# RHnejad/3D_PoseEstimation

Hardware: AMD Instinct MI355X
Metric: poses/sec fwd+bwd, 17-joint lifting batch 4096; MPJPE vs ref (higher is better)
Workload: dtype f16x3 (two fp16 planes per fp32 operand, 3 fp16 MFMAs per product, fp32 accumulate); 1 GPU; BASELINE configs[1]: phase1_lifting LinearModel 34-1024-2x(1024-1024)-51, BN+ReLU+Dropout(0.5), one train_1.py step = zero_grad+forward+MSE+backward+AdamW; launch=hipgraph (one hipGraph replay per step), per_gpu_batch=4096, global_batch=4096, parallelism=dp1

## Files before the change

3d_poseestimation_amd/_lib.py:

```python
import ctypes
import os

import torch

_HERE = os.path.dirname(os.path.abspath(__file__))
LIB_PATH = os.environ.get("POSELIFT_LIB") or os.path.join(_HERE, "csrc", "libposelift.so")

PL_F32, PL_BF16, PL_BF16X6, PL_F16X3 = 0, 1, 2, 3


GATHER_FN = ctypes.CFUNCTYPE(ctypes.c_int, ctypes.c_void_p, ctypes.c_void_p, ctypes.c_int64, ctypes.c_void_p)


class PLSync(ctypes.Structure):
    _fields_ = [("world", ctypes.c_int32), ("rank", ctypes.c_int32), ("gather", GATHER_FN),
                ("user", ctypes.c_void_p)]


class PLL1Term(ctypes.Structure):
    _fields_ = [("a", ctypes.c_void_p), ("b", ctypes.c_void_p), ("n", ctypes.c_int64),
                ("da", ctypes.c_void_p), ("db", ctypes.c_void_p)]


L1_MAX_TERMS = 8
# ... 40 lines not shown
_D = ctypes.POINTER(PLDesc)
SIGNATURES = {
    "pl_version": (_c.c_int, []),
    "pl_last_error": (_c.c_char_p, []),
    "pl_num_hidden": (_c.c_int64, [_D]),
    "pl_param_tensors": (_c.c_int64, [_D]),
    "pl_param_offset": (_c.c_int64, [_D, _c.c_int64]),
    "pl_param_numel": (_c.c_int64, [_D, _c.c_int64]),
    "pl_param_arena_floats": (_c.c_int64, [_D]),
    "pl_workspace_bytes": (_c.c_size_t, [_D, _c.c_int64]),
    "pl_workspace_view": (_c.c_int, [_D, _c.c_int64, _c.c_int, _c.c_int64,
                                     _c.POINTER(_c.c_size_t), _c.POINTER(_c.c_size_t)]),
    "pl_workspace_bitmap_format": (_c.c_int, [_D, _c.c_int64, _c.c_int64]),
    "pl_lifter_fwd_eval": (_c.c_int, [_D, _P, _P, _c.c_int64, _P, _c.c_size_t, _P]),
    "pl_lifter_fwd_train": (_c.c_int, [_D, _P, _P, _c.c_int64, _P, _c.c_size_t, _c.c_uint64,
                                       _c.c_uint64, _P, _P]),
    "pl_lifter_bwd": (_c.c_int, [_D, _P, _P, _c.c_int64, _P, _c.c_size_t, _P, _P, _P]),
    "pl_lifter_fwd_eval_saved": (_c.c_int, [_D, _P, _P, _c.c_int64, _P, _c.c_size_t, _P]),
    "pl_lifter_bwd_eval": (_c.c_int, [_D, _P, _P, _c.c_int64, _P, _c.c_size_t, _P, _P, _P]),
    "pl_lifter_bwd_layers": (_c.c_int, [_D, _P, _P, _c.c_int64, _P, _c.c_size_t, _P, _P, _c.c_int, _c.c_int, _P]),
    "pl_lifter_train_fwd_bwd": (_c.c_int, [_D, _P, _P, _c.c_int64, _P, _c.c_size_t, _c.c_uint64, _c.c_uint64,
                                           _P, _P, _P, _c.c_int, _c.c_int, _P]),
    "pl_lifter_step_carries_adamw": (_c.c_int, [_D, _c.c_int64]),
    "pl_lifter_train_step": (_c.c_int, [_D, _P, _P, _c.c_int64, _P, _c.c_size_t, _c.c_uint64, _c.c_uint64,
                                        _P, _P, _P, _c.POINTER(PLAdamWStep), _P]),
    "pl_mse_scratch_bytes": (_c.c_size_t, [_c.c_int64]),
    "pl_mse_fwd_bwd": (_c.c_int, [_P, _P, _c.c_int64, _c.c_float, _P, _P, _P, _P]),
    "pl_l1_scratch_bytes": (_c.c_size_t, [_c.c_int]),
    "pl_l1_terms_fwd_bwd": (_c.c_int, [_c.POINTER(PLL1Term), _c.c_int, _c.c_float, _P, _P, _P]),
    "pl_mpjpe_scratch_bytes": (_c.c_size_t, [_c.c_int64, _c.c_int64]),
    "pl_mpjpe_accum": (_c.c_int, [_P, _P, _c.c_int64, _c.c_int64, _P, _P, _P]),
    "pl_adamw_flat": (_c.c_int, [_P, _P, _P, _P, _c.c_int64, _c.c_float, _c.c_float, _c.c_float,
                                 _c.c_float, _c.c_float, _c.c_int64, _c.c_float, _P]),
    "pl_adamw_flat_dev": (_c.c_int, [_P, _P, _P, _P, _c.c_int64, _P, _c.c_float, _c.c_float, _c.c_float,
                                     _c.c_float, _c.c_int64, _P, _c.c_float, _P]),
    "pl_adamw_flat_planes": (_c.c_int, [_P, _P, _P, _P, _c.c_int64, _c.c_float, _P, _c.c_float, _c.c_float, _c.c_float,
                                        _c.c_float, _c.c_int64, _P, _c.c_float, _c.POINTER(PLAdamWPlanes), _P]),
    "pl_wplanes_bytes": (_c.c_size_t, [_D]),
    "pl_wplanes_layer_bytes": (_c.c_size_t, [_D]),
    "pl_weight_plane_scale": (_c.c_float, []),
    "pl_wplanes_refresh": (_c.c_int, [_D, _P]),
    "pl_flip_pose": (_c.c_int, [_P, _P, _c.c_int64, _c.c_int64, _c.c_int64, _P]),
    "pl_counter_add": (_c.c_int, [_P, _c.c_int64, _P]),
    "pl_flip_pose_ex": (_c.c_int, [_P, _P, _P, _c.c_int64, _c.c_int64, _c.c_int64, _c.c_float, _c.c_float, _P]),
    "pl_flip_w_nhwc": (_c.c_int, [_P, _P, _c.c_int64, _c.c_int64, _c.c_int64, _c.c_int64, _P]),
    "pl_softargmax3d_nhwc_fwd": (_c.c_int, [_P, _c.c_int64, _c.c_int64, _c.c_int64, _c.c_int64, _P, _P, _P]),
# ... 178 lines not shown
```

3d_poseestimation_amd/csrc/api.hip:

```cpp
#include <stdarg.h>
#include <stdio.h>
#include <stdlib.h>

#include <vector>

#include "adamw.h"
#include "pl_internal.h"

namespace pl {

static thread_local char g_err[512] = "";

void set_error(const char* fmt, ...) {
  va_list ap;
  va_start(ap, fmt);
  vsnprintf(g_err, sizeof(g_err), fmt, ap);
  va_end(ap);
}

namespace {

inline int64_t align_up(int64_t v, int64_t a) { return (v + a - 1) / a * a; }

int check_desc(const PLDesc* d, bool need_arenas) {
// ... 107 lines not shown
  bool bnr_fused;
};
enum class Loss : uint8_t { SmallMse, FromSlabs, PartialOnly };

struct Ws {
  int L, G, RC;
  std::vector<size_t> z, act, bits, mean, rstd, dbpart;
  size_t stat, scale, shift, coef, ga, gb, dz, slabs, outpart, dyout, mse, total;
  size_t act_bytes, bits_bytes;
  size_t slab_floats;
  bool planes;
  int pkind;
  std::vector<size_t> actp, wp;
  std::vector<size_t> sactp;
  std::vector<char> act_f32;
  size_t dzp, amax, dzscale;
  size_t skp_out, skp_in;
  std::vector<size_t> wslab;
  std::vector<LayerRoute> layer;
  bool bn_small;
  bool small_layer;
  bool top_fused;
  bool adam_rides;
  bool small_f16;
  bool eval_small;
  bool out_narrow;
  bool out_skinny;
  Loss loss;
};

Ws plan(const PLDesc* d, int64_t B) {
  Ws w;
  w.L = 1 + 2 * d->num_stage;
  const int H = d->hidden;
  w.G = gemm_stat_groups((int)B);
  w.RC = bwd_row_chunks((int)B, H);
  size_t o = 0;
  auto take = [&](size_t bytes) {
    const size_t at = o;
    o = (size_t)align_up((int64_t)(o + bytes), 256);
    return at;
  };
  w.act_bytes = (size_t)B * H * sizeof(float);
  w.bits_bytes = std::max((size_t)B * bitmap_words_per_row(H), (size_t)H) * sizeof(uint64_t);
  w.pkind = planes_kind(d, B);
  w.planes = w.pkind != 0;
// ... 41 lines not shown
  w.skp_out = take((size_t)skinny_in_chunks((int)B) * d->out_dim * H * 4);
  w.skp_in = take((size_t)skinny_in_chunks((int)B) * d->in_dim * H * 4);
  if (w.planes) {
    w.wslab.push_back(0);
    for (int l = 1; l < w.L; ++l) w.wslab.push_back(take((size_t)tn_splits(H, H, (int)B) * H * H * 4));
    for (int l = 0; l + 1 < w.L; ++l) w.actp.push_back(take(w.act_bytes));
    w.wp.push_back(0);
    for (int l = 1; l < w.L; ++l) w.wp.push_back(take((size_t)H * H * 4));
    w.dzp = take(w.act_bytes);
    w.amax = take(std::max((size_t)((H + 255) / 256) * w.RC, (size_t)(B / 64) * (H / 32)) * 2 * 4);
    w.dzscale = take((size_t)w.L * 2 * 4);
  }
  if (d->dtype == PL_F16X3 && B <= kThinGemmMaxM)
    for (int l = 0; l + 1 < w.L; ++l) w.sactp.push_back(take(w.act_bytes));
  w.total = o;

  const int world = sync_world(d);
  const bool first_ok = small_first_ok(d->in_dim), mid_ok = B * world <= 512 && small_layer_ok(2, H, H);
  w.bn_small = d->bn && !w.planes && world == 1 && B >= 2 && B <= kBnSmallRows;
  w.small_layer = w.bn_small && small_layer_ok((int)B, H, H);
  w.top_fused = w.small_layer && small_top_ok(d->out_dim);
  const bool small_head = w.top_fused && (d->num_stage > 0 || first_ok);
  w.adam_rides = small_head && H % 128 == 0;
  w.small_f16 = d->dtype == PL_F16X3 && !w.sactp.empty() && first_ok;
  w.eval_small = d->bn && B <= kThinGemmMaxM && small_layer_ok(2, H, H) && first_ok && small_top_ok(d->out_dim);
  w.out_narrow = skinny_narrow_out_supported(H, d->out_dim);
  w.out_skinny = skinny_supported(d->out_dim, H);
  const int so = w.out_narrow ? skinny_narrow_out_splits((int)B, H) : 0;
  w.loss = small_head ? Loss::SmallMse : (so && mse_from_slabs_supported(so, d->out_dim)) ? Loss::FromSlabs : Loss::PartialOnly;
  for (int l = 0; l < w.L; ++l) {
    LayerRoute r;
    if (l == 0) r.lin = skinny_supported(d->in_dim, H) ? Lin::Skinny : Lin::Gemm;
    else if (w.planes) r.lin = w.pkind == 2 && mid_ok ? Lin::PlanesMid : Lin::Planes;
    else r.lin = d->bn && d->dtype != PL_BF16 && B > kBnSmallRows && mid_ok ? Lin::F32Mid : Lin::Gemm;
    r.groups = r.lin == Lin::Skinny ? skinny_stat_groups((int)B) : w.G;
    const bool tile = w.small_layer && (l > 0 || first_ok);
    if (!d->bn) r.stats = Stats::None;
    else if (w.bn_small) r.stats = tile ? Stats::InLayer : Stats::Small;
    else r.stats = world == 1 && r.groups >= 1 && r.groups <= 4 ? Stats::InApply : Stats::Finalize;
    if (l == 0) r.bwd = tile && w.L > 1 ? Bwd::InAbove : Bwd::First;
    else if (!w.small_layer) r.bwd = w.planes ? Bwd::PlanesPair : Bwd::F32Pair;
    else r.bwd = H % 128 == 0 ? Bwd::SmallLayerDw : Bwd::SmallLayer;
    r.bnr_fused = w.planes && (l < w.L - 1 || w.out_skinny);
    w.layer.push_back(r);
  }
  return w;
// ... 388 lines not shown
  const int H = d->hidden, O = d->out_dim, Bi = (int)B;
  const float kscale = (!eval_bn && d->p_dropout > 0.f && d->p_dropout < 1.f) ? 1.0f / (1.0f - d->p_dropout) : 1.0f;
  float* slabs = f32(ws, w.slabs);
  float* GA = f32(ws, w.ga);
  float* GB = f32(ws, w.gb);
  float* DZ = f32(ws, w.dz);
  const int64_t BH = B * H;
  const int n_amax = ((H + 255) / 256) * w.RC;
  std::vector<const float*> jpart; std::vector<float*> jout; std::vector<int> jR, jH, jkind, jtrans;
  auto job = [&](const float* part, float* out, int R, int Hj, int kind, int transK) {
    jpart.push_back(part); jout.push_back(out); jR.push_back(R); jH.push_back(Hj); jkind.push_back(kind); jtrans.push_back(transK);
  };

  const bool small = !eval_bn && w.bn_small, sl = !eval_bn && w.small_layer;
  auto bn_layer = [&](int l) {
    const Layer y = layer_of(d, P, grads, l);
    SmallBnLayer b = {f32(ws, w.z[l]), f32(ws, w.mean[l]), f32(ws, w.rstd[l]), y.gamma, u64(ws, w.bits[l]),
                      w.layer[l].stats != Stats::InLayer, y.ggamma, y.gbeta, y.gb};
    return b;
  };
  const int n_loss_part = loss_partials > 0 ? loss_partials : mse_partials(B * O);
  const bool top_fused = do_output && !eval_bn && w.top_fused && l_hi == w.L - 1 && l_hi >= l_lo;
  const bool adam_rides = adam && top_fused && l_lo == 0 && w.adam_rides;
  auto ride = [&](int64_t lo, int64_t hi) {
    AdamWRide r = {};
    r.p = const_cast<float*>(d->params) + lo; r.g = grads + lo; r.m = adam->m + lo; r.v = adam->v + lo; r.n = hi - lo;
    r.lr = adam->lr; r.beta1 = adam->beta1; r.beta2 = adam->beta2; r.eps = adam->eps; r.wd = adam->weight_decay; r.gscale = 1.0f;
    r.t = adam->t; r.lr_dev = adam->lr_dev; r.t_dev = adam->t_dev;
    return r;
  };
  if (top_fused) {
    PL_TRY(launch_small_top_bwd(dy, d->params + P.off[4 * w.L], f32(ws, w.act[w.L - 1]), Bi, H, O, GA, grads + P.off[4 * w.L],
                                grads + P.off[4 * w.L + 1], bn_layer(w.L - 1), kscale, DZ, s, f32(ws, w.mse),
                                n_loss_part, 1.0f / (float)(B * O), loss_out, const_cast<uint64_t*>(d->step_dev)));
  } else if (do_output && w.out_skinny) {
    PL_TRY(launch_skinny_wide_in(dy, f32(ws, w.act[w.L - 1]), grads + P.off[4 * w.L], Bi, O, H, false, f32(ws, w.skp_out), s,
                                 false, f32(ws, w.outpart)));
    job(f32(ws, w.skp_out), grads + P.off[4 * w.L], skinny_in_chunks(Bi), O * H, 0, 0);
    job(f32(ws, w.outpart), grads + P.off[4 * w.L + 1], skinny_in_chunks(Bi), O, 0, 0);
    GemmArgs be = {};
    const int lt = w.L - 1;
    if (!eval_bn && w.layer[lt].bnr_fused) {
      const BnrSlab sl = bnr_slab(d, w, ws, Bi / 64, (w.pkind == 2 && lt > 0) ? (Bi / 64) * (H / 32) : 0, eval_bn);
      be.bnr_z = f32(ws, w.z[lt]); be.bnr_bits = u64(ws, w.bits[lt]);
      be.bnr_mean = f32(ws, w.mean[lt]); be.bnr_rstd = f32(ws, w.rstd[lt]); be.bnr_kscale = kscale;
      be.bnr_part_dy = sl.mine; be.bnr_part_dyz = sl.mine + (size_t)(Bi / 64) * H;
// ... 51 lines not shown
    const float* a_in = l == 0 ? x : (w.planes ? nullptr : f32(ws, w.act[l - 1]));
    if (pl_layer) {
      const int splits = tn_splits(H, H, Bi);
      PlanesGemmArgs nn = planes_args(w.pkind, u16(ws, w.dzp), BH, H, wplane(d, w, ws, l), (int64_t)H * H, H,
                                      (l % 2 == 1) ? GA : GB, Bi, H, H, 1.0f / kWeightPlaneScale, dzs ? dzs + 1 : nullptr);
      if (l % 2 == 1) nn.e.addend = GA;
      if (!eval_bn && w.layer[l - 1].bnr_fused) {
        const bool lower_scaled = w.pkind == 2 && l - 1 > 0;
        const BnrSlab sl = bnr_slab(d, w, ws, Bi / 64, lower_scaled ? (Bi / 64) * (H / 64) : 0, eval_bn);
        nn.e.bnr_z = f32(ws, w.z[l - 1]);
        nn.e.bnr_bits = u64(ws, w.bits[l - 1]);
        nn.e.bnr_mean = f32(ws, w.mean[l - 1]);
        nn.e.bnr_rstd = f32(ws, w.rstd[l - 1]);
        nn.e.bnr_kscale = kscale;
        nn.e.bnr_part_dy = sl.mine;
        nn.e.bnr_part_dyz = sl.mine + (size_t)(Bi / 64) * H;
        nn.e.bnr_amax = lower_scaled ? sl.amax_mine : nullptr;
      }
      float* wsl = f32(ws, w.wslab[l]);
      PlanesGemmArgs tn = planes_args(w.pkind, u16(ws, w.dzp), BH, H, u16(ws, w.actp[l - 1]), BH, H,
                                      splits > 1 ? wsl : ly.gW, H, H, Bi, 1.0f / kActPlaneScale, dzs ? dzs + 1 : nullptr);
      tn.e.split_k = splits;
      PL_TRY(launch_gemm_planes_pair(nn, tn, s));
      if (splits > 1) job(wsl, ly.gW, splits, H * H, 1, 0);
    } else if (l > 0) {
      GemmArgs g = {};
      g.A = DZl; g.B = ly.W; g.M = Bi; g.N = H; g.K = H; g.lda = H; g.ldb = H; g.ldc = H; g.split_k = 1;
      if (l % 2 == 1) { g.C = GA; g.addend = GA; } else { g.C = GB; }
      g.arith = arith_of(d);
      g.thin_scratch = slabs; g.thin_scratch_floats = w.slab_floats;
      GemmArgs t = {};
      t.arith = g.arith;
      t.A = DZl; t.B = a_in; t.M = H; t.N = H; t.K = Bi; t.lda = H; t.ldb = H; t.ldc = H; t.split_k = 1; t.C = ly.gW;
      if (sl && (r.bwd == Bwd::SmallLayer || r.bwd == Bwd::SmallLayerDw)) {
        const bool dw_rides = r.bwd == Bwd::SmallLayerDw;
        if (l - 1 >= l_lo) {
          const bool w1 = l == 1 && w.layer[0].bwd == Bwd::InAbove;
          AdamWRide ar = {};
          if (adam_rides) ar = ride(P.off[4 * l + 1], l == w.L - 1 ? P.total : P.off[4 * (l + 1) + 1]);
          PL_TRY(launch_small_layer_bwd(DZl, ly.W, (l % 2 == 1) ? GA : nullptr, (l % 2 == 1) ? GA : nullptr, Bi, H, H,
                                        bn_layer(l - 1), kscale, dzbuf(l - 1), s, dw_rides ? a_in : nullptr,
                                        dw_rides ? ly.gW : nullptr, w1 ? x : nullptr, w1 ? grads + P.off[0] : nullptr, d->in_dim,
                                        adam_rides ? &ar : nullptr));
          if (dw_rides) continue;
        } else {
          PL_TRY(launch_gemm_f32(kNN, g, s));
        }
// ... 12 lines not shown
      PL_TRY(gemm_tn_reduced(DZ, H, a_in, ly.K, ly.gW, H, ly.K, Bi, slabs, s));
    }
    if (l == 0 && dx) {
      GemmArgs g = {};
      g.A = DZ; g.B = ly.W; g.C = dx; g.M = Bi; g.N = d->in_dim; g.K = H; g.lda = H; g.ldb = d->in_dim;
      g.ldc = d->in_dim; g.split_k = 1;
      PL_TRY(launch_gemm_f32(kNN, g, s));
    }
  }
  float inv_n = 0.f;
  uint64_t* tick = nullptr;
  if (loss_out && !top_fused) {
    const int64_t n = B * O;
    job(f32(ws, w.mse), loss_out, n_loss_part, 1, 2, 0);
    inv_n = 1.0f / (float)n;
    tick = const_cast<uint64_t*>(d->step_dev);
  }
  if (!jpart.empty())
    PL_TRY(launch_reduce_rows_multi(jpart.data(), jR.data(), jH.data(), jout.data(), (int)jpart.size(), s, jkind.data(),
                                    jtrans.data(), inv_n, tick));
  if (adam) {
    const int64_t n = adam_rides ? (w.L > 1 ? P.off[4 * 1 + 1] : P.total) : P.total;
    float* p = const_cast<float*>(d->params);
    if (adam->lr_dev)
      PL_TRY(pl_adamw_flat_dev(p, grads, adam->m, adam->v, n, adam->lr_dev, adam->beta1, adam->beta2, adam->eps,
                               adam->weight_decay, adam->t, adam->t_dev, 1.0f, stream));
    else
      PL_TRY(pl_adamw_flat(p, grads, adam->m, adam->v, n, adam->lr, adam->beta1, adam->beta2, adam->eps, adam->weight_decay,
                           adam->t, 1.0f, stream));
  }
  return PL_OK;
}

extern "C" int pl_lifter_bwd(const PLDesc* d, const float* x, const float* dy, int64_t B, void* ws,
                             size_t ws_bytes, float* dx, float* grads, void* stream) {
  if (!d) PL_FAIL(PL_EINVAL, "descriptor is NULL");
  return bwd_impl(d, x, dy, B, ws, ws_bytes, dx, grads, stream, true, 2 * d->num_stage, 0);
}

extern "C" int pl_lifter_bwd_eval(const PLDesc* d, const float* x, const float* dy, int64_t B, void* ws,
                                  size_t ws_bytes, float* dx, float* grads, void* stream) {
  if (!d) PL_FAIL(PL_EINVAL, "descriptor is NULL");
  return bwd_impl(d, x, dy, B, ws, ws_bytes, dx, grads, stream, true, 2 * d->num_stage, 0, true);
}

static int check_range(const PLDesc* d, int hi, int lo, const char* who) {
// ... 256 lines not shown
  return launch_planes_split_k("pl_conv2d_planes_wgrad", kTN, g, dw, slabs, (hipStream_t)stream);
}

extern "C" int pl_prof_enable(int on) { return prof_enable(on); }
extern "C" int pl_prof_read(double min_flops, double max_flops, double* ms_total, int64_t* launches,
                            double* flops_total) {
  if (!ms_total || !launches || !flops_total) PL_FAIL(PL_EINVAL, "pl_prof_read: null pointer");
  return prof_read(min_flops, max_flops, ms_total, launches, flops_total);
}

static int train_fwd_bwd_impl(const PLDesc* d, const float* x, const float* target, int64_t B, void* ws, size_t ws_bytes,
                              uint64_t seed, uint64_t step, float* y, float* loss, float* grads, int hi, int lo, void* stream,
                              const PLAdamWStep* adam);

extern "C" int pl_lifter_train_fwd_bwd(const PLDesc* d, const float* x, const float* target, int64_t B, void* ws,
                                       size_t ws_bytes, uint64_t seed, uint64_t step, float* y, float* loss,
                                       float* grads, int hi, int lo, void* stream) {
  return train_fwd_bwd_impl(d, x, target, B, ws, ws_bytes, seed, step, y, loss, grads, hi, lo, stream, nullptr);
}

extern "C" int pl_lifter_step_carries_adamw(const PLDesc* d, int64_t B) {
  PL_TRY(check_desc(d, false));
  return B > 0 && plan(d, B).adam_rides ? 1 : 0;
}

extern "C" int pl_lifter_train_step(const PLDesc* d, const float* x, const float* target, int64_t B, void* ws, size_t ws_bytes,
                                    uint64_t seed, uint64_t step, float* y, float* loss, float* grads, const PLAdamWStep* opt,
                                    void* stream) {
  if (!opt || !opt->m || !opt->v || (opt->lr_dev != nullptr) != (opt->t_dev != nullptr) || opt->t < (opt->t_dev ? 0 : 1))
    PL_FAIL(PL_EINVAL, "pl_lifter_train_step: bad optimizer description");
  if (!d) PL_FAIL(PL_EINVAL, "descriptor is NULL");
  return train_fwd_bwd_impl(d, x, target, B, ws, ws_bytes, seed, step, y, loss, grads, 1 + 2 * d->num_stage, 0, stream, opt);
}

static int train_fwd_bwd_impl(const PLDesc* d, const float* x, const float* target, int64_t B, void* ws, size_t ws_bytes,
                              uint64_t seed, uint64_t step, float* y, float* loss, float* grads, int hi, int lo, void* stream,
                              const PLAdamWStep* adam) {
  PL_TRY(check_desc(d, true));
  if (!x || !target || !y || !loss || !grads) PL_FAIL(PL_EINVAL, "pl_lifter_train_fwd_bwd: null pointer");
  if (B <= 0) PL_FAIL(PL_ESHAPE, "pl_lifter_train_fwd_bwd: B=%lld", (long long)B);
  PL_TRY(check_range(d, hi, lo, "pl_lifter_train_fwd_bwd"));
  const Ws w = plan(d, B);
  PL_TRY(check_ws(w, ws, ws_bytes));
  float* dy = f32(ws, w.dyout);
  const int L = 1 + 2 * d->num_stage;
  if (hi == L && w.loss == Loss::PartialOnly) {
// ... 16 lines not shown
```

3d_poseestimation_amd/csrc/elementwise.hip:

```cpp
#include "adamw.h"
#include "bn_pieces.h"
#include "philox.h"
#include <stdlib.h>

#include "pl_internal.h"
#include "plane_store.h"

namespace pl {
namespace {

constexpr int NTHR = 256;

__device__ __forceinline__ float4 ld4(const float* p) { return *reinterpret_cast<const float4*>(p); }
__device__ __forceinline__ void st4(float* p, float4 v) { *reinterpret_cast<float4*>(p) = v; }

__global__ __launch_bounds__(256) void split_planes_kernel(const float* __restrict__ x, int64_t n4, PlaneOut o) {
  const PlaneDst d = plane_dst(o);
  const int64_t stride = (int64_t)gridDim.x * blockDim.x;
  for (int64_t i = (int64_t)blockIdx.x * blockDim.x + threadIdx.x; i < n4; i += stride)
    store_planes4(d, (size_t)i * 4, ld4(x + 4 * i));
}

struct Strided4 { int d1, d2, d3; int64_t s0, s1, s2, s3; };
__global__ __launch_bounds__(256) void split_planes_strided_kernel(const float* __restrict__ x, Strided4 v, int64_t n4, PlaneOut o) {
// ... 1182 lines not shown
      adamw_one(pv.x, gv.x, mv.x, vv.x, k);
      adamw_one(pv.y, gv.y, mv.y, vv.y, k);
      adamw_one(pv.z, gv.z, mv.z, vv.z, k);
      adamw_one(pv.w, gv.w, mv.w, vv.w, k);
      st4(p + 4 * i, pv); st4(m + 4 * i, mv); st4(v + 4 * i, vv);
      if (in.nseg) {
        const int64_t e = 4 * i;
#pragma unroll 1
        for (int q = 0; q < in.nseg; ++q) {
          const int64_t r = e - in.seg_off[q];
          if (r >= 0 && r < in.seg_n[q]) {
            const PlaneDst d = {in.seg_h[q], in.seg_l[q], in.pscale, in.kind};
            store_planes4(d, (size_t)r, pv);
            break;
          }
        }
      }
    }
    i = (n4 << 2) + (int64_t)blockIdx.x * blockDim.x + threadIdx.x;
  }
  for (; i < n; i += stride) adamw_one(p[i], g[i], m[i], v[i], k);
}

inline bool aligned16(const void* p) { return (reinterpret_cast<uintptr_t>(p) & 15) == 0; }
inline int stream_rows_grid(int B, int strips) {
  int gy = (2048 + strips - 1) / strips;
  const int need = (B + 3) / 4;
  if (gy > need) gy = need;
  return gy < 1 ? 1 : gy;
}

}

__global__ __launch_bounds__(NTHR) void bn_merge_groups_kernel(const float* __restrict__ in, int G, int rows, int H, int F,
                                                               float* __restrict__ out, int Gp) {
  const int c = blockIdx.x * NTHR + threadIdx.x;
  if (c >= H) return;
  const int gp = blockIdx.y;
  const size_t GH = (size_t)G * H;
  float S = 0.f, Q = 0.f, na = 0.f;
  for (int f0 = 0; f0 < F; f0 += 8) {
    float s[8], q[8], n[8];
#pragma unroll
    for (int u = 0; u < 8; ++u) {
      const int g = gp * F + f0 + u;
      n[u] = (f0 + u < F && g < G) ? (float)max(0, min(64, rows - 64 * g)) : 0.f;
// ... 358 lines not shown
}

static AdamWIn adamw_in(float lr, float beta1, float beta2, float eps, float wd, float gscale, int64_t t,
                        const float* lr_dev, const uint64_t* t_dev) {
  AdamWIn in = {};
  in.lr = lr; in.beta1 = beta1; in.beta2 = beta2; in.eps = eps; in.wd = wd; in.gscale = gscale; in.t = t;
  in.lr_dev = lr_dev; in.t_dev = t_dev;
  return in;
}

extern "C" int pl_adamw_flat(float* p, const float* g, float* m, float* v, int64_t n, float lr,
                             float beta1, float beta2, float eps, float weight_decay, int64_t t,
                             float grad_scale, void* stream) {
  return adamw_launch(p, g, m, v, n, adamw_in(lr, beta1, beta2, eps, weight_decay, grad_scale, t, nullptr, nullptr), stream);
}

extern "C" int pl_adamw_flat_dev(float* p, const float* g, float* m, float* v, int64_t n, const float* lr_dev,
                                 float beta1, float beta2, float eps, float weight_decay, int64_t t_base,
                                 const uint64_t* t_dev, float grad_scale, void* stream) {
  if (!lr_dev || !t_dev) PL_FAIL(PL_EINVAL, "pl_adamw_flat_dev: null lr / t pointer");
  return adamw_launch(p, g, m, v, n, adamw_in(0.f, beta1, beta2, eps, weight_decay, grad_scale, t_base, lr_dev, t_dev), stream);
}

extern "C" int pl_adamw_flat_planes(float* p, const float* g, float* m, float* v, int64_t n, float lr, const float* lr_dev,
                                    float beta1, float beta2, float eps, float weight_decay, int64_t t,
                                    const uint64_t* t_dev, float grad_scale, const PLAdamWPlanes* planes, void* stream) {
  if ((lr_dev != nullptr) != (t_dev != nullptr)) PL_FAIL(PL_EINVAL, "pl_adamw_flat_planes: lr_dev and t_dev go together");
  AdamWIn in = adamw_in(lr, beta1, beta2, eps, weight_decay, grad_scale, t, lr_dev, t_dev);
  if (planes && planes->nseg > 0) {
    if (planes->nseg > PL_ADAMW_MAX_SEGS || (planes->kind != 1 && planes->kind != 2) || !(planes->scale > 0.f))
      PL_FAIL(PL_EINVAL, "pl_adamw_flat_planes: bad plane description");
    if (!(aligned16(p) && aligned16(g) && aligned16(m) && aligned16(v)) || (n & 3))
      PL_FAIL(PL_EINVAL, "pl_adamw_flat_planes: arenas must be 16-byte aligned, n %% 4 == 0");
    in.nseg = planes->nseg; in.kind = planes->kind; in.pscale = planes->scale;
    for (int q = 0; q < planes->nseg; ++q) {
      const PLAdamWSeg& sg = planes->seg[q];
      if (sg.offset < 0 || sg.numel <= 0 || (sg.offset & 3) || (sg.numel & 3) || sg.offset + sg.numel > n || !sg.h ||
          (planes->kind == 2 && !sg.l) || (reinterpret_cast<uintptr_t>(sg.h) & 7) || (reinterpret_cast<uintptr_t>(sg.l) & 7))
        PL_FAIL(PL_EINVAL, "pl_adamw_flat_planes: segment %d", q);
      in.seg_off[q] = sg.offset; in.seg_n[q] = sg.numel;
      in.seg_h[q] = static_cast<unsigned short*>(sg.h); in.seg_l[q] = static_cast<unsigned short*>(sg.l);
    }
  }
  return adamw_launch(p, g, m, v, n, in, stream);
}

__global__ void counter_add_kernel(uint64_t* counter, int64_t delta) { counter[0] = (uint64_t)((int64_t)counter[0] + delta); }
extern "C" int pl_counter_add(uint64_t* counter, int64_t delta, void* stream) {
  if (!counter) PL_FAIL(PL_EINVAL, "pl_counter_add: null counter");
  hipLaunchKernelGGL(counter_add_kernel, dim3(1), dim3(1), 0, (hipStream_t)stream, counter, delta);
  PL_CHECK_LAUNCH("counter_add");
  return PL_OK;
}

extern "C" int pl_flip_pose(const float* in, float* out, int64_t B, int64_t joints, int64_t D, void* stream) {
  if (!in || !out || in == out) PL_FAIL(PL_EINVAL, "pl_flip_pose: null or aliased pointers");
  if (B <= 0 || joints != 17 || (D != 2 && D != 3)) PL_FAIL(PL_ESHAPE, "pl_flip_pose: expects (B, 17, 2|3)");
  const int64_t n = B * joints * D;
  hipLaunchKernelGGL(flip_pose_kernel, dim3((unsigned)((n + NTHR - 1) / NTHR)), dim3(NTHR), 0, (hipStream_t)stream,
                     in, out, n, (int)D);
  PL_CHECK_LAUNCH("flip_pose");
  return PL_OK;
}

extern "C" int pl_flip_tta_pack(const float* x, float* xx, int64_t B, int64_t joints, int64_t D, void* stream) {
  if (!x || !xx) PL_FAIL(PL_EINVAL, "pl_flip_tta_pack: null pointer");
  if (B <= 0 || joints != 17 || (D != 2 && D != 3)) PL_FAIL(PL_ESHAPE, "pl_flip_tta_pack: expects (B, 17, 2|3)");
// ... 276 lines not shown
```

3d_poseestimation_amd/csrc/pl_internal.h:

```cpp
#pragma once
#include <hip/hip_runtime.h>
#include <stddef.h>
#include <stdint.h>

#include "../../include/poselift.h"

namespace pl {

constexpr int kWave = 64;

void set_error(const char* fmt, ...);

#define PL_FAIL(code, ...)        \
  do {                            \
    ::pl::set_error(__VA_ARGS__); \
    return (code);                \
  } while (0)

#define PL_CHECK_LAUNCH(what)                                              \
  do {                                                                     \
    hipError_t e__ = hipGetLastError();                                    \
    if (e__ != hipSuccess)                                                 \
      PL_FAIL(PL_EHIP, "%s: launch failed: %s", what, hipGetErrorString(e__)); \
  } while (0)
// ... 148 lines not shown
  const float *z, *mean, *rstd, *gamma;
  const uint64_t* bits;
  bool rowbits;
  float *dgamma, *dbeta, *dbias;
};
int launch_small_layer_bwd(const float* dz, const float* W, const float* addend, float* gout, int B, int H, int K,
                           const SmallBnLayer& below, float kscale, float* dz_lo, hipStream_t s, const float* a_in = nullptr,
                           float* dW = nullptr, const float* x1 = nullptr, float* dW1 = nullptr, int K1 = 0,
                           const struct AdamWRide* adam = nullptr);
int launch_small_top_bwd(const float* dy, const float* W2, const float* h, int B, int H, int O, float* gout, float* dW2,
                         float* db2, const SmallBnLayer& top, float kscale, float* dz_top, hipStream_t s,
                         const float* mpart = nullptr, int np = 0, float inv_n = 0.f, float* loss = nullptr,
                         uint64_t* tick = nullptr);
int launch_bn_eval_stats(const float* gamma, const float* beta, const float* rm, const float* rv, float eps, int H,
                         float* mean, float* rstd, float* scale, float* shift, hipStream_t s);
int launch_bn_bwd_dz(const float* g, const uint64_t* bits, const float* z, const float* mean,
                     const float* rstd, const float* coef, float keep_scale, int bn, int B, int H,
                     float* dz, float* part_db, hipStream_t s, int Hc = 0, const PlaneOut* planes = nullptr, int rc = 0);

int launch_reduce_slabs(const float* slabs, int nslab, int64_t n, float* out, hipStream_t s);
int launch_reduce_rows_multi(const float* const* part, const int* R, const int* H, float* const* out, int njobs,
                             hipStream_t s, const int* kind = nullptr, const int* transK = nullptr, float loss_inv_n = 0.f,
                             uint64_t* loss_tick = nullptr);
int mse_partial_only(const float* pred, const float* tgt, int64_t n, float grad_scale, float* dpred, void* scratch, void* stream);
int mse_partials(int64_t n);
bool mse_from_slabs_supported(int splits, int N);
int mse_partial_from_slabs(const float* part, int splits, int B, int N, const float* bias, const float* tgt, float grad_scale,
                           float* y, float* dpred, void* scratch, void* stream);
int launch_reduce_slabs_bias(const float* slabs, int nslab, int rows, int cols, const float* bias,
                             float* out, hipStream_t s);
int colsum_chunks(int rows);
int launch_colsum_partial(const float* X, int rows, int cols, float* part, hipStream_t s);
int launch_bn_fold_eval(const float* bias, const float* gamma, const float* beta, const float* rm,
                        const float* rv, float eps, int bn, int H, float* scale, float* shift,
                        hipStream_t s);
int launch_fill(float* p, int64_t n, float v, hipStream_t s);

bool skinny_supported(int K, int H);
int skinny_chunks(int B);
int skinny_stat_groups(int B);
int launch_skinny_wide_out(const float* X, const float* W, const float* bias, float* out, int B, int K,
                           int H, bool w_transposed, float* stat_sum, float* stat_m2, hipStream_t s,
                           const GemmArgs* bnr = nullptr);
int launch_skinny_wide_in(const float* X, const float* D, float* out, int B, int K, int H,
                          bool out_transposed, float* part, hipStream_t s, bool reduce = true, float* xsum = nullptr);
int skinny_in_chunks(int B);
// ... 8 lines not shown
```

3d_poseestimation_amd/model.py:

```python
import ctypes
import weakref

import torch
from torch import nn
from torch.autograd.graph import increment_version

from . import _lib
from .layout import bitmap_words_per_row, hidden_layer_prefixes, param_slots


class Linear(nn.Module):

    def __init__(self, linear_size, p_dropout=0.5, BN=True):
        super().__init__()
        self.l_size = linear_size
        self.w1 = nn.Linear(linear_size, linear_size)
        self.batch_norm1 = nn.BatchNorm1d(linear_size)
        self.w2 = nn.Linear(linear_size, linear_size)
        self.batch_norm2 = nn.BatchNorm1d(linear_size)
        self.BN = BN

    def forward(self, x):
        raise _lib.PoseliftError("residual blocks are evaluated by LinearModel.forward as one fused path")

# ... 393 lines not shown
                self._guarded(ws, lambda: _lib.lib().pl_lifter_bwd_layers(*args, hi, lo, _lib.current_stream_ptr()),
                              "pl_lifter_bwd_layers")
                sync.launch_bucket(target[a_lo:a_hi])
        elif eval_mode:
            self._guarded(ws, lambda: _lib.lib().pl_lifter_bwd_eval(*args, _lib.current_stream_ptr()), "pl_lifter_bwd_eval")
        else:
            self._guarded(ws, lambda: _lib.lib().pl_lifter_bwd(*args, _lib.current_stream_ptr()), "pl_lifter_bwd")
        if accumulate:
            for s, p in zip(self._slots, self._param_list):
                gview = target[s.offset:s.offset + s.numel].view(s.shape)
                if p.grad is None:
                    p.grad = gview.clone()
                else:
                    p.grad.add_(gview)
        else:
            for s, p in zip(self._slots, self._param_list):
                if self.BN or "batch_norm" not in s.name:
                    p.grad = target[s.offset:s.offset + s.numel].view(s.shape)
        return dx

    def step_carries_adamw(self, B):
        return _lib.lib().pl_lifter_step_carries_adamw(ctypes.byref(self._desc), int(B)) == 1

    def fused_train_fwd_bwd(self, x2, target, sync=None, step_dev=None, adamw=None):
        B = x2.shape[0]
        ws = self._acquire_workspace(B)
        try:
            y = torch.empty(B, self.output_size, dtype=torch.float32, device=x2.device)
            loss = torch.empty((), dtype=torch.float32, device=x2.device)
            grads = self.flat_grads
            self._step += 1
            L = _lib.lib()
            self._desc.step_dev = step_dev.data_ptr() if step_dev is not None else None
            if adamw is not None and self.step_carries_adamw(B):
                self._desc.wplanes_valid = 0
            else:
                self._mark_wplanes()

            def call(hi, lo):
                self._guarded(ws, lambda: L.pl_lifter_train_fwd_bwd(
                    ctypes.byref(self._desc), x2.data_ptr(), target.data_ptr(), B, ws["buf"].data_ptr(), ws["bytes"],
                    self._seed, self._step, y.data_ptr(), loss.data_ptr(), grads.data_ptr(), hi, lo,
                    _lib.current_stream_ptr()), "pl_lifter_train_fwd_bwd")
            if adamw is not None:
                if sync is not None:
                    raise _lib.PoseliftError("fused_train_fwd_bwd: the in-call AdamW step and a gradient sync exclude each other")
                self._guarded(ws, lambda: L.pl_lifter_train_step(
                    ctypes.byref(self._desc), x2.data_ptr(), target.data_ptr(), B, ws["buf"].data_ptr(), ws["bytes"],
                    self._seed, self._step, y.data_ptr(), loss.data_ptr(), grads.data_ptr(), ctypes.byref(adamw),
                    _lib.current_stream_ptr()), "pl_lifter_train_step")
            elif sync is not None and sync.world() > 1 and _overlap_ok(sync):
                for hi, lo, a_lo, a_hi in self._bwd_ranges():
                    call(hi, lo)
                    sync.launch_bucket(grads[a_lo:a_hi])
            else:
                call(len(self._named_holders()), 0)
            increment_version(self._arena_tensors if adamw is not None else self._bn_buffers)
        finally:
            self._desc.step_dev = None
            self._release_workspace(ws)
        if self._param_list[-1].grad is None or self._param_list[-1].grad.data_ptr() != \
                grads.data_ptr() + 4 * self._slots[-1].offset:
            for s, p in zip(self._slots, self._param_list):
                p.grad = grads[s.offset:s.offset + s.numel].view(s.shape) if (self.BN or "batch_norm" not in s.name) else None
        self.last_workspace = ws
        return loss, y

    def forward(self, x):
        if not self._arenas_intact():
            self._flatten()
        B = x.shape[0]
        x2 = x.reshape(B, -1)
        if x2.shape[1] != self.input_size:
            raise ValueError(f"expected {self.input_size} input features, got {x2.shape[1]}")
        if x2.dtype != torch.float32:
            x2 = x2.float()
        x2 = x2.contiguous()
        _lib.require_device_tensor(x2, "x")
        _lib.require_device_tensor(self._flat, "parameters")
        if x2.device != self._flat.device:
# ... 31 lines not shown
```

3d_poseestimation_amd/train.py:

```python
import torch
from torch.autograd.graph import increment_version

from . import _lib


class _MSEFn(torch.autograd.Function):

    @staticmethod
    def forward(ctx, pred, tgt):
        _lib.require_device_tensor(pred, "pred")
        _lib.require_device_tensor(tgt, "target")
        if pred.shape != tgt.shape:
            raise ValueError(f"MSE shapes differ: {tuple(pred.shape)} vs {tuple(tgt.shape)}")
        n = pred.numel()
        need = pred.requires_grad
        dpred = torch.empty_like(pred) if need else None
        loss = torch.empty((), dtype=torch.float32, device=pred.device)
        scratch = torch.empty(_lib.lib().pl_mse_scratch_bytes(n), dtype=torch.uint8, device=pred.device)
        with _lib.on_device(pred.device):
            rc = _lib.lib().pl_mse_fwd_bwd(pred.data_ptr(), tgt.data_ptr(), n, 1.0,
                                           dpred.data_ptr() if need else None, loss.data_ptr(),
                                           scratch.data_ptr(), _lib.current_stream_ptr())
        _lib.check(rc, "pl_mse_fwd_bwd")
        ctx.dpred = dpred
# ... 82 lines not shown
        rc = _lib.lib().pl_flip_w_nhwc(f.data_ptr(), out.data_ptr(), f.shape[0], f.shape[1], f.shape[2], f.shape[3],
                                       _lib.current_stream_ptr())
    _lib.check(rc, "pl_flip_w_nhwc")
    return out


def epoch_mpjpe_mm(metric_sum, n_samples, num_of_joints=17, zero_centre=True):
    m = torch.mean((metric_sum / n_samples)[1:17])
    if num_of_joints == 17 and zero_centre:
        m = m * (17 / 16) * 1000
    return m


def _fusable(model, optimizer, y1, y2):
    from .model import LinearModel
    from .optim import FlatAdamW
    return (isinstance(model, LinearModel) and isinstance(optimizer, FlatAdamW) and optimizer._model is model
            and model.training and torch.is_grad_enabled() and not y1.requires_grad and y1.is_cuda and y2.is_cuda
            and model._inject_keep is None and model._arenas_intact()
            and y2.numel() == y2.shape[0] * model.output_size
            and y1.numel() == y1.shape[0] * model.input_size)


def train_step(model, optimizer, y1, y2, grad_sync=None):
    y1, y2 = y1.float(), y2.float()
    if _fusable(model, optimizer, y1, y2):
        with _lib.on_device(y1.device):
            x2, t2 = y1.reshape(y1.shape[0], -1).contiguous(), y2.reshape(y2.shape[0], -1).contiguous()
            if grad_sync is None and model._grad_sync is None and model.step_carries_adamw(x2.shape[0]):
                adamw = optimizer._step_struct(float(optimizer.param_groups[0]["lr"]), None, optimizer._t + 1, None)
                if adamw is not None:
                    loss, y2_hat = model.fused_train_fwd_bwd(x2, t2, None, adamw=adamw)
                    optimizer._advance_host(1)
                    return loss, y2_hat.reshape(y2.shape)
            loss, y2_hat = model.fused_train_fwd_bwd(x2, t2, grad_sync if model._grad_sync is grad_sync else None)
        optimizer.step(grad_scale=grad_sync(model) if grad_sync is not None else 1.0)
        return loss, y2_hat.reshape(y2.shape)
    optimizer.zero_grad()
    y2_hat = model(y1).reshape(y2.shape)
    loss = mse_loss(y2_hat, y2)
    loss.backward()
    if grad_sync is not None:
        optimizer.step(grad_scale=grad_sync(model))
    else:
        optimizer.step()
    return loss, y2_hat


class GraphedTrainStep:

    def __init__(self, model, optimizer, y1, y2):
        y1, y2 = y1.float(), y2.float()
# ... 2 lines not shown
                                     "and no gradient sync attached")
        self.model, self.opt = model, optimizer
        B = y1.shape[0]
        dev = y1.device
        self._x = y1.reshape(B, -1).contiguous().clone()
        self._y = y2.reshape(B, -1).contiguous().clone()
        self._out_shape = tuple(y2.shape)
        self._tick = torch.zeros(1, dtype=torch.int64, device=dev)
        self._lr = float(optimizer.param_groups[0]["lr"])
        self._lr_dev = torch.full((1,), self._lr, dtype=torch.float32, device=dev)
        optimizer._bind()
        with _lib.on_device(dev):
            snap = [t.clone() for t in (model.flat_params, model._bn_running, model._bn_batches, optimizer._m, optimizer._v)]
            step0, t0 = model._step, optimizer._t
            train_step(model, optimizer, self._x, self._y.reshape(self._out_shape))
            for dst, src in zip((model.flat_params, model._bn_running, model._bn_batches, optimizer._m, optimizer._v), snap):
                dst.copy_(src)
            model._step, optimizer._t = step0, t0
            optimizer._step_tensor.fill_(float(t0))
            increment_version(model._arena_tensors)
            model._ensure_wplanes()
            torch.cuda.synchronize(dev)
            self.graph = torch.cuda.CUDAGraph()
            adamw = optimizer._step_struct(0.0, self._lr_dev, t0, self._tick) if model.step_carries_adamw(B) else None
            self._in_call = adamw is not None
            with torch.cuda.graph(self.graph):
                if adamw is not None:
                    self.loss, y_hat = model.fused_train_fwd_bwd(self._x, self._y, None, step_dev=self._tick, adamw=adamw)
                    self._refreshes_planes = False
                else:
                    self.loss, y_hat = model.fused_train_fwd_bwd(self._x, self._y, None, step_dev=self._tick)
                    self._refreshes_planes = optimizer._enqueue_dev(self._lr_dev, t0, self._tick)
            self.y_hat = y_hat.reshape(self._out_shape)
            model._step = step0
        self._step0, self._t0, self._seed0, self.replays = step0, t0, model._seed, 0
        self._ptrs = self._baked_ptrs()

    @property
    def inputs(self):
        return self._x, self._y

    def _baked_ptrs(self):
        return (self.model.flat_params.data_ptr(), self.opt._m.data_ptr() if self.opt._m is not None else 0,
                self.opt._v.data_ptr() if self.opt._v is not None else 0)

    def __call__(self, y1, y2):
        lr = float(self.opt.param_groups[0]["lr"])
        if lr != self._lr:
            self._lr = lr
            self._lr_dev.fill_(lr)
        ds, dt = self.model._step - self._step0, self.opt._t - self._t0
        if self.model._seed != self._seed0 or self._baked_ptrs() != self._ptrs:
# ... 151 lines not shown
```

include/poselift.h:

```cpp
#ifndef POSELIFT_H_
#define POSELIFT_H_

#include <stddef.h>
#include <stdint.h>

#ifdef __cplusplus
extern "C" {
#endif

#define PL_VERSION 111

typedef enum PLStatus {
  PL_OK = 0,
  PL_EINVAL = -1,
  PL_ESHAPE = -2,
  PL_EDTYPE = -3,
  PL_EBATCH = -4,
  PL_EHIP = -5,
  PL_EWORKSPACE = -6,
  PL_ESYNC = -7
} PLStatus;

typedef enum PLDtype { PL_F32 = 0, PL_BF16 = 1, PL_BF16X6 = 2, PL_F16X3 = 3 } PLDtype;

typedef int (*PLGatherFn)(void* user, float* buf, int64_t floats_per_rank, void* stream);
typedef struct PLSync {
  int32_t world;
  int32_t rank;
  PLGatherFn gather;
  void* user;
} PLSync;

typedef struct PLDesc {
// ... 45 lines not shown
int pl_lifter_fwd_eval_saved(const PLDesc* d, const float* x, float* y, int64_t B,
                             void* workspace, size_t workspace_bytes, void* stream);
int pl_lifter_bwd_eval(const PLDesc* d, const float* x, const float* dy, int64_t B,
                       void* workspace, size_t workspace_bytes, float* dx, float* flat_grads, void* stream);

int pl_lifter_bwd_layers(const PLDesc* d, const float* x, const float* dy, int64_t B,
                         void* workspace, size_t workspace_bytes, float* dx,
                         float* flat_grads, int hi, int lo, void* stream);

int pl_lifter_train_fwd_bwd(const PLDesc* d, const float* x, const float* target, int64_t B,
                            void* workspace, size_t workspace_bytes, uint64_t seed, uint64_t step,
                            float* y, float* loss, float* flat_grads, int hi, int lo, void* stream);

typedef struct PLAdamWStep {
  float* m;
  float* v;
  float lr;
  const float* lr_dev;
  float beta1, beta2, eps, weight_decay;
  int64_t t;
  const uint64_t* t_dev;
} PLAdamWStep;
int pl_lifter_step_carries_adamw(const PLDesc* d, int64_t B);
int pl_lifter_train_step(const PLDesc* d, const float* x, const float* target, int64_t B, void* workspace,
                         size_t workspace_bytes, uint64_t seed, uint64_t step, float* y, float* loss, float* flat_grads,
                         const PLAdamWStep* opt, void* stream);

int pl_softargmax3d_nhwc_fwd(const float* logits, int64_t B, int64_t J, int64_t H, int64_t W,
                             float* coords, float* stats, void* stream);
int pl_softargmax3d_nhwc_bwd(const float* logits, const float* stats, const float* gcoords, int64_t B, int64_t J,
                             int64_t H, int64_t W, float* dlogits, void* stream);

size_t pl_conv2d_nhwc_scratch_bytes(int64_t B, int64_t H, int64_t W, int64_t Cin, int64_t Cout, int KH,
                                    int KW, int stride, int pad);
size_t pl_conv2d_nhwc_scratch_bytes_ex(int64_t B, int64_t H, int64_t W, int64_t Cin, int64_t Cout, int KH,
                                       int KW, int stride, int pad, int has_bias, int has_resid, int relu);
int pl_conv2d_nhwc_fwd(const float* x, int64_t B, int64_t H, int64_t W, int64_t Cin, const float* w,
                       int64_t Cout, int KH, int KW, int stride, int pad, const float* scale,
                       const float* shift, const float* bias, int relu, const float* resid, float* y,
                       int arith, void* scratch, size_t scratch_bytes, void* stream);

size_t pl_conv2d_nhwc_wgrad_scratch_bytes(int64_t B, int64_t H, int64_t W, int64_t Cin, int64_t Cout,
                                          int KH, int KW, int stride, int pad);
int pl_conv2d_nhwc_wgrad(const float* x, int64_t B, int64_t H, int64_t W, int64_t Cin, const float* dy,
                         int64_t Cout, int KH, int KW, int stride, int pad, float* dw, int arith, void* scratch,
                         size_t scratch_bytes, void* stream);
// ... 224 lines not shown
```

Measured before the change: 6.726 million poses/s.

## Fold split-K weight-gradient slab reduction into the AdamW update kernel

When weight planes are in use and the split-K count is small, the hidden-layer weight-gradient slabs are no longer reduced by a separate job. The AdamW kernel sums the slabs while reading gradients, writes the summed gradient back, updates the parameters and refreshes the fp16 weight planes in the same pass. The captured graph then carries the optimizer step inside the fused train call. This removes one full-size gradient write and read plus a launch. In exchange, AdamW does a per-element segment lookup and extra slab loads, and the Python side has to track plane versioning for the new path.

Measured after the change: 6.711 million poses/s (median of 2 runs). No clear change (-0.2%).

```diff
diff --git a/3d_poseestimation_amd/_lib.py b/3d_poseestimation_amd/_lib.py
--- a/3d_poseestimation_amd/_lib.py
+++ b/3d_poseestimation_amd/_lib.py
@@ -86,6 +86,7 @@
     "pl_lifter_train_fwd_bwd": (_c.c_int, [_D, _P, _P, _c.c_int64, _P, _c.c_size_t, _c.c_uint64, _c.c_uint64,
                                            _P, _P, _P, _c.c_int, _c.c_int, _P]),
     "pl_lifter_step_carries_adamw": (_c.c_int, [_D, _c.c_int64]),
+    "pl_lifter_step_sums_slabs": (_c.c_int, [_D, _c.c_int64]),
     "pl_lifter_train_step": (_c.c_int, [_D, _P, _P, _c.c_int64, _P, _c.c_size_t, _c.c_uint64, _c.c_uint64,
                                         _P, _P, _P, _c.POINTER(PLAdamWStep), _P]),
     "pl_mse_scratch_bytes": (_c.c_size_t, [_c.c_int64]),
diff --git a/3d_poseestimation_amd/csrc/api.hip b/3d_poseestimation_amd/csrc/api.hip
--- a/3d_poseestimation_amd/csrc/api.hip
+++ b/3d_poseestimation_amd/csrc/api.hip
@@ -153,6 +153,7 @@
   bool small_layer;
   bool top_fused;
   bool adam_rides;
+  bool adam_sums_slabs;
   bool small_f16;
   bool eval_small;
   bool out_narrow;
@@ -240,6 +241,7 @@
   w.top_fused = w.small_layer && small_top_ok(d->out_dim);
   const bool small_head = w.top_fused && (d->num_stage > 0 || first_ok);
   w.adam_rides = small_head && H % 128 == 0;
+  w.adam_sums_slabs = w.planes && world == 1 && tn_splits(H, H, (int)B) <= kAdamWMaxSlabs && w.L - 1 <= PL_ADAMW_MAX_SEGS;
   w.small_f16 = d->dtype == PL_F16X3 && !w.sactp.empty() && first_ok;
   w.eval_small = d->bn && B <= kThinGemmMaxM && small_layer_ok(2, H, H) && first_ok && small_top_ok(d->out_dim);
   w.out_narrow = skinny_narrow_out_supported(H, d->out_dim);
@@ -674,6 +676,8 @@
   const int n_loss_part = loss_partials > 0 ? loss_partials : mse_partials(B * O);
   const bool top_fused = do_output && !eval_bn && w.top_fused && l_hi == w.L - 1 && l_hi >= l_lo;
   const bool adam_rides = adam && top_fused && l_lo == 0 && w.adam_rides;
+  const bool adam_sums_slabs = adam && !adam_rides && !eval_bn && do_output && l_hi == w.L - 1 && l_lo == 0 && w.adam_sums_slabs;
+  AdamWSlabSegs slab_segs = {};
   auto ride = [&](int64_t lo, int64_t hi) {
     AdamWRide r = {};
     r.p = const_cast<float*>(d->params) + lo; r.g = grads + lo; r.m = adam->m + lo; r.v = adam->v + lo; r.n = hi - lo;
@@ -771,7 +775,13 @@
                                       splits > 1 ? wsl : ly.gW, H, H, Bi, 1.0f / kActPlaneScale, dzs ? dzs + 1 : nullptr);
       tn.e.split_k = splits;
       PL_TRY(launch_gemm_planes_pair(nn, tn, s));
-      if (splits > 1) job(wsl, ly.gW, splits, H * H, 1, 0);
+      if (splits > 1 && adam_sums_slabs) {
+        const int q = slab_segs.nseg++;
+        slab_segs.S = splits;
+        slab_segs.off[q] = P.off[4 * l]; slab_segs.numel[q] = (int64_t)H * H; slab_segs.slab[q] = wsl;
+      } else if (splits > 1) {
+        job(wsl, ly.gW, splits, H * H, 1, 0);
+      }
     } else if (l > 0) {
       GemmArgs g = {};
       g.A = DZl; g.B = ly.W; g.M = Bi; g.N = H; g.K = H; g.lda = H; g.ldb = H; g.ldc = H; g.split_k = 1;
@@ -830,6 +840,17 @@
   if (adam) {
     const int64_t n = adam_rides ? (w.L > 1 ? P.off[4 * 1 + 1] : P.total) : P.total;
     float* p = const_cast<float*>(d->params);
+    if (adam_sums_slabs) {
+      PLAdamWPlanes planes = {};
+      if (d->wplanes) {
+        planes.kind = w.pkind; planes.scale = kWeightPlaneScale;
+        for (int l = 1; l < w.L; ++l) {
+          unsigned short* q = wplane(d, w, ws, l);
+          planes.seg[planes.nseg++] = PLAdamWSeg{P.off[4 * l], (int64_t)H * H, q, w.pkind == 2 ? q + (size_t)H * H : nullptr};
+        }
+      }
+      return launch_adamw_flat_slabs(p, grads, adam->m, adam->v, P.total, *adam, slab_segs, d->wplanes ? &planes : nullptr, s);
+    }
     if (adam->lr_dev)
       PL_TRY(pl_adamw_flat_dev(p, grads, adam->m, adam->v, n, adam->lr_dev, adam->beta1, adam->beta2, adam->eps,
                                adam->weight_decay, adam->t, adam->t_dev, 1.0f, stream));
@@ -1132,6 +1153,11 @@
 extern "C" int pl_lifter_step_carries_adamw(const PLDesc* d, int64_t B) {
   PL_TRY(check_desc(d, false));
   return B > 0 && plan(d, B).adam_rides ? 1 : 0;
+}
+
+extern "C" int pl_lifter_step_sums_slabs(const PLDesc* d, int64_t B) {
+  PL_TRY(check_desc(d, false));
+  return B > 0 && plan(d, B).adam_sums_slabs ? 1 : 0;
 }
 
 extern "C" int pl_lifter_train_step(const PLDesc* d, const float* x, const float* target, int64_t B, void* ws, size_t ws_bytes,
diff --git a/3d_poseestimation_amd/csrc/elementwise.hip b/3d_poseestimation_amd/csrc/elementwise.hip
--- a/3d_poseestimation_amd/csrc/elementwise.hip
+++ b/3d_poseestimation_amd/csrc/elementwise.hip
@@ -1228,6 +1228,57 @@
   for (; i < n; i += stride) adamw_one(p[i], g[i], m[i], v[i], k);
 }
 
+__global__ __launch_bounds__(NTHR) void adamw_slabs_kernel(float* __restrict__ p, float* __restrict__ g, float* __restrict__ m,
+                                                           float* __restrict__ v, int64_t n4, AdamWIn in, AdamWSlabSegs sl) {
+  const AdamWK k = adamw_consts(in);
+  const int64_t stride = (int64_t)gridDim.x * blockDim.x;
+  for (int64_t i = (int64_t)blockIdx.x * blockDim.x + threadIdx.x; i < n4; i += stride) {
+    const int64_t e = 4 * i;
+    float4 pv = ld4(p + e), mv = ld4(m + e), vv = ld4(v + e);
+    const float* __restrict__ sp = nullptr;
+    int64_t sn = 0;
+#pragma unroll 1
+    for (int q = 0; q < sl.nseg; ++q) {
+      const int64_t r = e - sl.off[q];
+      if (r >= 0 && r < sl.numel[q]) { sp = sl.slab[q] + r; sn = sl.numel[q]; break; }
+    }
+    float4 gv;
+    if (sp) {
+      gv = ld4(sp);
+      const float4 b1 = ld4(sp + sn);
+      if (sl.S == 4) {
+        const float4 b2 = ld4(sp + 2 * sn), b3 = ld4(sp + 3 * sn);
+        gv.x += b1.x; gv.y += b1.y; gv.z += b1.z; gv.w += b1.w;
+        gv.x += b2.x; gv.y += b2.y; gv.z += b2.z; gv.w += b2.w;
+        gv.x += b3.x; gv.y += b3.y; gv.z += b3.z; gv.w += b3.w;
+      } else if (sl.S == 3) {
+        const float4 b2 = ld4(sp + 2 * sn);
+        gv.x += b1.x; gv.y += b1.y; gv.z += b1.z; gv.w += b1.w;
+        gv.x += b2.x; gv.y += b2.y; gv.z += b2.z; gv.w += b2.w;
+      } else {
+        gv.x += b1.x; gv.y += b1.y; gv.z += b1.z; gv.w += b1.w;
+      }
+      st4(g + e, gv);
+    } else {
+      gv = ld4(g + e);
+    }
+    adamw_one(pv.x, gv.x, mv.x, vv.x, k);
+    adamw_one(pv.y, gv.y, mv.y, vv.y, k);
+    adamw_one(pv.z, gv.z, mv.z, vv.z, k);
+    adamw_one(pv.w, gv.w, mv.w, vv.w, k);
+    st4(p + e, pv); st4(m + e, mv); st4(v + e, vv);
+#pragma unroll 1
+    for (int q = 0; q < in.nseg; ++q) {
+      const int64_t r = e - in.seg_off[q];
+      if (r >= 0 && r < in.seg_n[q]) {
+        const PlaneDst d = {in.seg_h[q], in.seg_l[q], in.pscale, in.kind};
+        store_planes4(d, (size_t)r, pv);
+        break;
+      }
+    }
+  }
+}
+
 inline bool aligned16(const void* p) { return (reinterpret_cast<uintptr_t>(p) & 15) == 0; }
 inline int stream_rows_grid(int B, int strips) {
   int gy = (2048 + strips - 1) / strips;
@@ -1632,11 +1683,43 @@
   return adamw_launch(p, g, m, v, n, adamw_in(0.f, beta1, beta2, eps, weight_decay, grad_scale, t_base, lr_dev, t_dev), stream);
 }
 
+static int adamw_set_planes(AdamWIn& in, const PLAdamWPlanes* planes, const float* p, const float* g, const float* m, const float* v,
+                            int64_t n);
+
 extern "C" int pl_adamw_flat_planes(float* p, const float* g, float* m, float* v, int64_t n, float lr, const float* lr_dev,
                                     float beta1, float beta2, float eps, float weight_decay, int64_t t,
                                     const uint64_t* t_dev, float grad_scale, const PLAdamWPlanes* planes, void* stream) {
   if ((lr_dev != nullptr) != (t_dev != nullptr)) PL_FAIL(PL_EINVAL, "pl_adamw_flat_planes: lr_dev and t_dev go together");
   AdamWIn in = adamw_in(lr, beta1, beta2, eps, weight_decay, grad_scale, t, lr_dev, t_dev);
+  PL_TRY(adamw_set_planes(in, planes, p, g, m, v, n));
+  return adamw_launch(p, g, m, v, n, in, stream);
+}
+
+int pl::launch_adamw_flat_slabs(float* p, float* g, float* m, float* v, int64_t n, const PLAdamWStep& step,
+                                const AdamWSlabSegs& segs, const PLAdamWPlanes* planes, hipStream_t s) {
+  if (!p || !g || !m || !v) PL_FAIL(PL_EINVAL, "adamw_flat_slabs: null pointer");
+  if (n <= 0 || (n & 3) || !(aligned16(p) && aligned16(g) && aligned16(m) && aligned16(v)))
+    PL_FAIL(PL_EINVAL, "adamw_flat_slabs: arenas must be 16-byte aligned, n %% 4 == 0");
+  if ((step.lr_dev != nullptr) != (step.t_dev != nullptr) || step.t < (step.t_dev ? 0 : 1))
+    PL_FAIL(PL_EINVAL, "adamw_flat_slabs: bad step description");
+  if (segs.nseg < 0 || segs.nseg > PL_ADAMW_MAX_SEGS || (segs.nseg > 0 && (segs.S < 2 || segs.S > kAdamWMaxSlabs)))
+    PL_FAIL(PL_EINVAL, "adamw_flat_slabs: %d ranges of %d slabs", segs.nseg, segs.S);
+  for (int q = 0; q < segs.nseg; ++q)
+    if (segs.off[q] < 0 || segs.numel[q] <= 0 || (segs.off[q] & 3) || (segs.numel[q] & 3) || segs.off[q] + segs.numel[q] > n ||
+        !segs.slab[q] || !aligned16(segs.slab[q]))
+      PL_FAIL(PL_EINVAL, "adamw_flat_slabs: range %d", q);
+  AdamWIn in = adamw_in(step.lr, step.beta1, step.beta2, step.eps, step.weight_decay, 1.0f, step.t, step.lr_dev, step.t_dev);
+  PL_TRY(adamw_set_planes(in, planes, p, g, m, v, n));
+  const int64_t n4 = n >> 2;
+  int blocks = (int)((n4 + NTHR - 1) / NTHR);
+  if (blocks > kAdamBlocks) blocks = kAdamBlocks;
+  hipLaunchKernelGGL(adamw_slabs_kernel, dim3(blocks), dim3(NTHR), 0, s, p, g, m, v, n4, in, segs);
+  PL_CHECK_LAUNCH("adamw_slabs");
+  return PL_OK;
+}
+
+static int adamw_set_planes(AdamWIn& in, const PLAdamWPlanes* planes, const float* p, const float* g, const float* m, const float* v,
+                            int64_t n) {
   if (planes && planes->nseg > 0) {
     if (planes->nseg > PL_ADAMW_MAX_SEGS || (planes->kind != 1 && planes->kind != 2) || !(planes->scale > 0.f))
       PL_FAIL(PL_EINVAL, "pl_adamw_flat_planes: bad plane description");
@@ -1652,7 +1735,7 @@
       in.seg_h[q] = static_cast<unsigned short*>(sg.h); in.seg_l[q] = static_cast<unsigned short*>(sg.l);
     }
   }
-  return adamw_launch(p, g, m, v, n, in, stream);
+  return PL_OK;
 }
 
 __global__ void counter_add_kernel(uint64_t* counter, int64_t delta) { counter[0] = (uint64_t)((int64_t)counter[0] + delta); }
diff --git a/3d_poseestimation_amd/csrc/pl_internal.h b/3d_poseestimation_amd/csrc/pl_internal.h
--- a/3d_poseestimation_amd/csrc/pl_internal.h
+++ b/3d_poseestimation_amd/csrc/pl_internal.h
@@ -194,6 +194,10 @@
 int launch_reduce_rows_multi(const float* const* part, const int* R, const int* H, float* const* out, int njobs,
                              hipStream_t s, const int* kind = nullptr, const int* transK = nullptr, float loss_inv_n = 0.f,
                              uint64_t* loss_tick = nullptr);
+constexpr int kAdamWMaxSlabs = 4;
+struct AdamWSlabSegs { int nseg, S; int64_t off[PL_ADAMW_MAX_SEGS], numel[PL_ADAMW_MAX_SEGS]; const float* slab[PL_ADAMW_MAX_SEGS]; };
+int launch_adamw_flat_slabs(float* p, float* g, float* m, float* v, int64_t n, const PLAdamWStep& step, const AdamWSlabSegs& segs,
+                            const PLAdamWPlanes* planes, hipStream_t s);
 int mse_partial_only(const float* pred, const float* tgt, int64_t n, float grad_scale, float* dpred, void* scratch, void* stream);
 int mse_partials(int64_t n);
 bool mse_from_slabs_supported(int splits, int N);
diff --git a/3d_poseestimation_amd/model.py b/3d_poseestimation_amd/model.py
--- a/3d_poseestimation_amd/model.py
+++ b/3d_poseestimation_amd/model.py
@@ -439,6 +439,9 @@
     def step_carries_adamw(self, B):
         return _lib.lib().pl_lifter_step_carries_adamw(ctypes.byref(self._desc), int(B)) == 1
 
+    def step_sums_slabs(self, B):
+        return _lib.lib().pl_lifter_step_sums_slabs(ctypes.byref(self._desc), int(B)) == 1
+
     def fused_train_fwd_bwd(self, x2, target, sync=None, step_dev=None, adamw=None):
         B = x2.shape[0]
         ws = self._acquire_workspace(B)
@@ -473,6 +476,8 @@
             else:
                 call(len(self._named_holders()), 0)
             increment_version(self._arena_tensors if adamw is not None else self._bn_buffers)
+            if adamw is not None and self._wplanes is not None and self.step_sums_slabs(B):
+                self._wplanes_ver = self._planes_key()
         finally:
             self._desc.step_dev = None
             self._release_workspace(ws)
diff --git a/3d_poseestimation_amd/train.py b/3d_poseestimation_amd/train.py
--- a/3d_poseestimation_amd/train.py
+++ b/3d_poseestimation_amd/train.py
@@ -128,12 +128,16 @@
             and y1.numel() == y1.shape[0] * model.input_size)
 
 
+def _step_in_call(model, B):
+    return model.step_carries_adamw(B) or model.step_sums_slabs(B)
+
+
 def train_step(model, optimizer, y1, y2, grad_sync=None):
     y1, y2 = y1.float(), y2.float()
     if _fusable(model, optimizer, y1, y2):
         with _lib.on_device(y1.device):
             x2, t2 = y1.reshape(y1.shape[0], -1).contiguous(), y2.reshape(y2.shape[0], -1).contiguous()
-            if grad_sync is None and model._grad_sync is None and model.step_carries_adamw(x2.shape[0]):
+            if grad_sync is None and model._grad_sync is None and _step_in_call(model, x2.shape[0]):
                 adamw = optimizer._step_struct(float(optimizer.param_groups[0]["lr"]), None, optimizer._t + 1, None)
                 if adamw is not None:
                     loss, y2_hat = model.fused_train_fwd_bwd(x2, t2, None, adamw=adamw)
@@ -182,12 +186,12 @@
             model._ensure_wplanes()
             torch.cuda.synchronize(dev)
             self.graph = torch.cuda.CUDAGraph()
-            adamw = optimizer._step_struct(0.0, self._lr_dev, t0, self._tick) if model.step_carries_adamw(B) else None
-            self._in_call = adamw is not None
+            adamw = optimizer._step_struct(0.0, self._lr_dev, t0, self._tick) if _step_in_call(model, B) else None
+            self._in_call = adamw is not None and model.step_carries_adamw(B)
             with torch.cuda.graph(self.graph):
                 if adamw is not None:
                     self.loss, y_hat = model.fused_train_fwd_bwd(self._x, self._y, None, step_dev=self._tick, adamw=adamw)
-                    self._refreshes_planes = False
+                    self._refreshes_planes = not self._in_call and model._wplanes is not None
                 else:
                     self.loss, y_hat = model.fused_train_fwd_bwd(self._x, self._y, None, step_dev=self._tick)
                     self._refreshes_planes = optimizer._enqueue_dev(self._lr_dev, t0, self._tick)
diff --git a/include/poselift.h b/include/poselift.h
--- a/include/poselift.h
+++ b/include/poselift.h
@@ -8,7 +8,7 @@
 extern "C" {
 #endif
 
-#define PL_VERSION 111
+#define PL_VERSION 112
 
 typedef enum PLStatus {
   PL_OK = 0,
@@ -100,6 +100,7 @@
   const uint64_t* t_dev;
 } PLAdamWStep;
 int pl_lifter_step_carries_adamw(const PLDesc* d, int64_t B);
+int pl_lifter_step_sums_slabs(const PLDesc* d, int64_t B);
 int pl_lifter_train_step(const PLDesc* d, const float* x, const float* target, int64_t B, void* workspace,
                          size_t workspace_bytes, uint64_t seed, uint64_t step, float* y, float* loss, float* flat_grads,
                          const PLAdamWStep* opt, void* stream);
```
